# haiciyang/LaDiffCodec

Hardware: AMD Instinct MI355X
Metric: audio-sec decoded / wall-sec, 16kHz 3kbps 50-step DDPM (higher is better)
Workload: dtype bf16; 1 GPU; LaDiffCodec 3 kbps, diff_dims=256, enc_ratios 8 4, 50-step DDPM, batch=32x2.4 s utterances per GPU; global_batch=32, latent_len=1200, denoise_steps=50, rccl_ranks=1, batches_in_flight=1, parallelism=dp1 (utterance-sharded, no data-path collective)

## Files before the change

ladiffcodec_amd/csrc/conv_lean.inc:

```

struct LeanTile { int m0, n0, sk_k, sk_tile, R_lo, nrows, u_begin, u_end; };
struct LeanGeom {
  const LeanTile* tiles;
  unsigned long long* stamps;
  int debug;
  int ln_off;
  int grid;
};

enum { LEAN_K3 = 0, LEAN_K1 = 1, LEAN_K1_LN = 2, LEAN_K4S2 = 3, LEAN_K7 = 4 };
enum { LEAN_EPI_PLAIN = 0, LEAN_EPI_RES = 1, LEAN_EPI_GN = 2, LEAN_EPI_GN_RES = 3, LEAN_EPI_QKV = 4 };

template <int TM, int KIND, bool RF>
struct LeanShape {
  static constexpr bool K3 = KIND == LEAN_K3, K4 = KIND == LEAN_K4S2, K7 = KIND == LEAN_K7;
  static constexpr bool TAPS = K3 || K4 || K7;
  static constexpr int TG = K3 ? 3 : (TAPS ? 4 : 1), KC = TAPS ? 1 : 2, NS = TG * KC, NSB = NS + (RF ? 1 : 0);
  static constexpr int NTAP = K7 ? 8 : TG;
  static constexpr int BM = TM * 64, BN = 64;
  static constexpr int PLANE_ROWS = K4 ? (TM == 2 ? 272 : 144) : (TAPS ? (TM == 2 ? 144 : 80) : BM);
  static constexpr int NAW = (PLANE_ROWS / 16 + 3) / 4;
  static constexpr int NAW0 = NAW > 3 ? 3 : NAW, NAW1 = NAW - NAW0;
  static constexpr int PLANE_BYTES = PLANE_ROWS * kRowBytes + kRowBytes;
  static constexpr int ZERO_OFF = PLANE_ROWS * kRowBytes;
  static constexpr int B_OFF = KC * PLANE_BYTES;
  static constexpr int STAGE_BYTES = B_OFF + NSB * BN * kRowBytes;
  static_assert(NAW >= 1 && NAW <= 5 && NAW1 <= 2 && NSB >= 2 && NSB <= 4, "runs of at most four copies per M0 write (13-bit immediate)");
};

template <int N>
__device__ __forceinline__ void lean_dma_run(const char* base, unsigned m0v, unsigned cnt, unsigned v0, unsigned v1, unsigned v2) {
  if constexpr (N == 1) {
    if (cnt != 0u) asm volatile("s_mov_b32 m0, %2\n\ts_nop 0\n\tglobal_load_lds_dwordx4 %0, %1" ::"v"(v0), "s"(base), "s"(m0v) : "memory");
  } else if constexpr (N == 2) {
    asm volatile("s_mov_b32 m0, %3\n\ts_cmp_lt_u32 %4, 1\n\ts_cbranch_scc1 .Lq%=\n\tglobal_load_lds_dwordx4 %0, %2\n\t"
                 "s_cmp_lt_u32 %4, 2\n\ts_cbranch_scc1 .Lq%=\n\tglobal_load_lds_dwordx4 %1, %2 offset:1024\n.Lq%=:"
                 ::"v"(v0), "v"(v1), "s"(base), "s"(m0v), "s"(cnt) : "memory", "scc");
  } else {
    asm volatile("s_mov_b32 m0, %4\n\ts_cmp_lt_u32 %5, 1\n\ts_cbranch_scc1 .Lq%=\n\tglobal_load_lds_dwordx4 %0, %3\n\t"
                 "s_cmp_lt_u32 %5, 2\n\ts_cbranch_scc1 .Lq%=\n\tglobal_load_lds_dwordx4 %1, %3 offset:1024\n\t"
                 "s_cmp_lt_u32 %5, 3\n\ts_cbranch_scc1 .Lq%=\n\tglobal_load_lds_dwordx4 %2, %3 offset:2048\n.Lq%=:"
                 ::"v"(v0), "v"(v1), "v"(v2), "s"(base), "s"(m0v), "s"(cnt) : "memory", "scc");
  }
}
template <int N>
__device__ __forceinline__ void lean_dma_all(const char* base, unsigned m0v, unsigned v0, unsigned v1, unsigned v2, unsigned v3) {
  if constexpr (N == 2) {
    asm volatile("s_mov_b32 m0, %3\n\ts_nop 0\n\tglobal_load_lds_dwordx4 %0, %2\n\tglobal_load_lds_dwordx4 %1, %2 offset:1024"
                 ::"v"(v0), "v"(v1), "s"(base), "s"(m0v) : "memory");
  } else if constexpr (N == 3) {
    asm volatile("s_mov_b32 m0, %4\n\ts_nop 0\n\tglobal_load_lds_dwordx4 %0, %3\n\tglobal_load_lds_dwordx4 %1, %3 offset:1024\n\t"
                 "global_load_lds_dwordx4 %2, %3 offset:2048"
                 ::"v"(v0), "v"(v1), "v"(v2), "s"(base), "s"(m0v) : "memory");
  } else {
    asm volatile("s_mov_b32 m0, %5\n\ts_nop 0\n\tglobal_load_lds_dwordx4 %0, %4\n\tglobal_load_lds_dwordx4 %1, %4 offset:1024\n\t"
                 "global_load_lds_dwordx4 %2, %4 offset:2048\n\tglobal_load_lds_dwordx4 %3, %4 offset:3072"
                 ::"v"(v0), "v"(v1), "v"(v2), "v"(v3), "s"(base), "s"(m0v) : "memory");
  }
}


__device__ __forceinline__ float lean_wave_sum(float v) {
  auto dpp = [](float x, auto ctrl) { return __int_as_float(__builtin_amdgcn_update_dpp(0, __float_as_int(x), decltype(ctrl)::value, 0xf, 0xf, true)); };
  v += dpp(v, std::integral_constant<int, 0xB1>());
  v += dpp(v, std::integral_constant<int, 0x4E>());
  v += dpp(v, std::integral_constant<int, 0x141>());
  v += dpp(v, std::integral_constant<int, 0x140>());
  const int iv = __float_as_int(v);
  return (__int_as_float(__builtin_amdgcn_readlane(iv, 0)) + __int_as_float(__builtin_amdgcn_readlane(iv, 16))) +
         (__int_as_float(__builtin_amdgcn_readlane(iv, 32)) + __int_as_float(__builtin_amdgcn_readlane(iv, 48)));
}

template <int G>
__device__ __forceinline__ float lean_group_sum(float v) {
  static_assert(G == 4 || G == 8, "quad or half row");
  auto dpp = [](float x, auto ctrl) { return __int_as_float(__builtin_amdgcn_update_dpp(0, __float_as_int(x), decltype(ctrl)::value, 0xf, 0xf, true)); };
  v += dpp(v, std::integral_constant<int, 0xB1>());
  v += dpp(v, std::integral_constant<int, 0x4E>());
  if constexpr (G == 8) v += dpp(v, std::integral_constant<int, 0x141>());
// ... 327 lines not shown
  const int b_first = (int)fdiv((unsigned)m0, a.lrows_div);
  const int b_last = (int)fdiv((unsigned)(min(m0 + BM, M) - 1), a.lrows_div);
  for (int bb = b_first; bb <= b_last; ++bb) {
    const int lo = bb * a.L_rows, hi = min(lo + a.L_rows, M);
    float ps = 0.f;
#pragma unroll
    for (int i = 0; i < TM; ++i)
#pragma unroll
      for (int r = 0; r < 16; ++r) {
        const int rl = (wm * TM + i) * 32 + (r & 3) + 8 * (r >> 2) + 4 * g;
        const int m = m0 + rl;
        const bool in = m >= lo && m < hi;
        if (wn == 0) {
          const unsigned short pb = in ? hw_bf16(__expf(fminf(acc[i][0][r], kLinattnKClamp))) : (unsigned short)0;
          ps += __uint_as_float((unsigned)pb << 16);
          spT[i32 * P + rl] = pb;
        } else {
          svT[i32 * P + rl] = in ? hw_bf16(acc[i][0][r]) : (unsigned short)0;
        }
      }
    float* wsb = a.qkv_ctx_ws + (size_t)bb * a.qkv_ctx_stride;
    if (wn == 0) {
      ps += __shfl_xor(ps, 32);
      if (lane < 32) atomicAdd(&wsb[HD + head * D + i32], ps);
    }
    __syncthreads();
    if (wave == 0) {
      f32x16 c;
#pragma unroll
      for (int r = 0; r < 16; ++r) c[r] = 0.f;
#pragma unroll
      for (int sx = 0; sx < BM / 16; ++sx) {
        const uint4 pa = *reinterpret_cast<const uint4*>(&spT[i32 * P + 16 * sx + 8 * g]);
        const uint4 vb = *reinterpret_cast<const uint4*>(&svT[i32 * P + 16 * sx + 8 * g]);
        mfma_step<__bf16>(c, pa, vb);
      }
      float* ctx = wsb + 2 * HD + (size_t)head * D * D;
#pragma unroll
      for (int r = 0; r < 16; ++r) {
        const int d = (r & 3) + 8 * (r >> 2) + 4 * g;
        atomicAdd(&ctx[d * D + i32], c[r]);
      }
    }
    __syncthreads();
  }
}

typedef const __attribute__((address_space(3))) u32x4_t* lds_u4_cptr;
__device__ __forceinline__ uint4 lean_lds16(unsigned addr) {
  const u32x4_t v = *reinterpret_cast<lds_u4_cptr>(addr);
  return make_uint4(v[0], v[1], v[2], v[3]);
}

template <typename T, int TM, int KIND, bool RF, int EPI, bool SK, int S = 2>
__global__ __launch_bounds__(256, S == 3 ? 2 : 3) void conv_lean_kernel(const ConvKArgs a, const LeanGeom g) {
  using SH = LeanShape<TM, KIND, RF>;
  static_assert(S == 2 || (S == 3 && !SH::K4 && !SH::K7 && SH::NAW1 == 0), "three stages: the k = 3 and 1x1 kinds (one window run per plane)");
  constexpr int TN = 1, WM = 2, WN = 2, NW = 4, TG = SH::TG, KC = SH::KC, NS = SH::NS, NSB = SH::NSB, NAW = SH::NAW;
  constexpr int BM = SH::BM, BN = SH::BN, STAGE = SH::STAGE_BYTES, PLANE = SH::PLANE_BYTES;
  constexpr int BKE = kRowBytes / (int)sizeof(T);
  constexpr bool LN = KIND == LEAN_K1_LN;
  constexpr unsigned kBias = 3072u;
  static_assert(!RF || SH::K3, "the folded 1x1 conv rides on a k = 3 unit");
  static_assert((!SH::K4 && !SH::K7) || (EPI <= LEAN_EPI_RES && (!SK || SH::K4)), "k = 4 / 7: plain and residual epilogues; k = 7 is never split");
  extern __shared__ __attribute__((aligned(16))) char smem[];
  typedef __attribute__((address_space(3))) void* lptr_t;
  const unsigned lds_base = (unsigned)(size_t)(lptr_t)smem;

  const int tid = (int)threadIdx.x, lane = tid & 63;
  const int wave = __builtin_amdgcn_readfirstlane(tid >> 6);
  const int wm = wave >> 1, wn = wave & 1;
  const unsigned bid = blockIdx.x;
  unsigned long long t_start = 0, t_pro = 0, t_loop = 0, t_tab = 0, t_dma = 0;
  GnStamp gst = {0ull, 0ull, 0ull, 0u};
  if (g.stamps) t_start = __builtin_amdgcn_s_memtime();
  unsigned long long* kst_slot = nullptr;
  if (a.kst) {
    kst_slot = a.kst + (size_t)(a.kst_step[1] & 2047) * a.kst_stride;
    if (tid == 0 && bid == 0) kst_slot[0] = (unsigned long long)wall_clock64();
  }
  if (g.debug & 8) return;
  typedef const __attribute__((address_space(4))) LeanTile* tile_cptr;
  const tile_cptr tp = (tile_cptr)(unsigned long long)g.tiles + bid;
  LeanTile tl;
  tl.m0 = tp->m0; tl.n0 = tp->n0; tl.sk_k = tp->sk_k; tl.sk_tile = tp->sk_tile; tl.R_lo = tp->R_lo; tl.nrows = tp->nrows; tl.u_begin = tp->u_begin; tl.u_end = tp->u_end;
  const int M = a.B * a.L_rows;
  const int m0 = tl.m0, n0 = tl.n0, R_lo = tl.R_lo, nrows = tl.nrows;

  const int r16 = lane >> 2;
  const unsigned gslot = (unsigned)(((lane & 3) ^ ((r16 >> 2) & 3)) << 4);
  const unsigned ldb1 = (unsigned)a.C1 * (unsigned)sizeof(T), ldb2 = (unsigned)a.C2 * (unsigned)sizeof(T);
  unsigned vw[NAW];
  auto window_offsets = [&](const unsigned ldb) {
#pragma unroll
    for (int i = 0; i < NAW; ++i) {
      int r = (wave * NAW + i) * 16 + r16;
      if (r >= nrows) r = 0;
      vw[i] = (unsigned)(R_lo + r) * ldb + gslot + kBias - (unsigned)(i < SH::NAW0 ? i : i - SH::NAW0) * 1024u;
    }
  };
  const unsigned wcnt = (unsigned)__builtin_amdgcn_readfirstlane(max(0, min(NAW, (nrows - wave * NAW * 16 + 15) >> 4)));
  const unsigned slab_bytes = (unsigned)a.n_pad * kRowBytes;
  unsigned vb[4] = {0u, 0u, 0u, 0u};
#pragma unroll
  for (int q = 0; q < NSB; ++q) {
    const unsigned slab = SH::TAPS ? (unsigned)q * slab_bytes : (unsigned)q * (unsigned)a.wtaps * slab_bytes;
    vb[q] = slab + (unsigned)(n0 + wave * 16 + r16) * kRowBytes + gslot + kBias - (unsigned)q * 1024u;
  }
  const int csw = a.C1 / BKE;
  const int pc0 = SH::K7 ? tl.u_begin >> 1 : tl.u_begin * KC;
  int pc = pc0;
  const char* xb;
  if (pc0 >= csw && a.C2 > 0) {
    xb = a.x2 + (size_t)(pc0 - csw) * kRowBytes - kBias;
    window_offsets(ldb2);
  } else {
    xb = a.x1 + (size_t)pc0 * kRowBytes - kBias;
    window_offsets(ldb1);
  }
  const unsigned chunk_w = (unsigned)a.wtaps * slab_bytes;
  const char* wb = a.w + (size_t)pc0 * chunk_w - kBias;
  const unsigned m0_win = lds_base + (unsigned)(wave * NAW * 1024);
  const unsigned m0_b = lds_base + (unsigned)(SH::B_OFF + wave * NSB * 1024);
  if (g.stamps) t_tab = __builtin_amdgcn_s_memtime();

  const unsigned wcnt0 = SH::NAW1 ? min(wcnt, (unsigned)SH::NAW0) : wcnt, wcnt1 = wcnt - wcnt0;
  auto issue = [&](const int st) {
#pragma unroll
    for (int kc = 0; kc < KC; ++kc) {
      lean_dma_run<SH::NAW0>(xb + kc * kRowBytes, m0_win + (unsigned)(st * STAGE + kc * PLANE), wcnt0, vw[0], vw[NAW > 1 ? 1 : 0], vw[NAW > 2 ? 2 : 0]);
      if constexpr (SH::NAW1 > 0)
        lean_dma_run<SH::NAW1>(xb + kc * kRowBytes, m0_win + (unsigned)(st * STAGE + kc * PLANE + SH::NAW0 * 1024), wcnt1, vw[NAW > 3 ? 3 : 0], vw[NAW > 4 ? 4 : 0], 0u);
    }
    if constexpr (SH::K7) {
      if (st == 0) {
        lean_dma_all<4>(wb, m0_b + (unsigned)(st * STAGE), vb[0], vb[1], vb[2], vb[3]);
        wb += (size_t)4 * slab_bytes;
        return;
      }
      lean_dma_all<4>(wb, m0_b + (unsigned)(st * STAGE), vb[0], vb[1], vb[2], vb[3] - 3u * slab_bytes);
    } else {
      lean_dma_all<NSB>(wb, m0_b + (unsigned)(st * STAGE), vb[0], vb[1], vb[2], vb[3]);
    }
    pc += KC;
    xb += KC * kRowBytes;
    wb += SH::K7 ? (size_t)3 * slab_bytes : (size_t)KC * chunk_w;
    if (pc == csw) {
      xb = a.x2 - kBias;
      window_offsets(ldb2);
    }
  };
  issue(0);
  if constexpr (S == 3) {
    if (tl.u_begin + 1 < tl.u_end && !(g.debug & 16)) issue(1);
  }
  if (g.stamps) t_dma = __builtin_amdgcn_s_memtime();
  LeanCols cl = {0.f, 0.f, 0.f, 1.f, 0.f};
  auto fetch_cols = [&]() {
    const int ecol = n0 + wn * 32 + (lane & 31);
    const bool ok = ecol < a.n;
    const int cc = ok ? ecol : 0;
    if (a.bias && ok) cl.bias = a.bias[ecol];
    if constexpr (EPI == LEAN_EPI_GN || EPI == LEAN_EPI_GN_RES) {
      cl.gam = a.gn_gamma[cc]; cl.bet = a.gn_beta[cc];
      if (a.gn_ss) { cl.sc = a.gn_ss[cc] + 1.0f; cl.sh = a.gn_ss[a.n + cc]; }
    }
  };
  if constexpr (!RF) fetch_cols();

  if constexpr (LN) {
    constexpr int TPR = NW * 64 / BM;
    constexpr int EPV = 16 / (int)sizeof(T);
    const int row = tid / TPR, part = tid - row * TPR;
    const int C = a.C1, nvec = C / EPV;
    const char* src = a.x1 + (size_t)min(m0 + row, M - 1) * C * sizeof(T);
    float sm = 0.f, sq = 0.f;
    const float2* rs = a.ln_rowstat ? reinterpret_cast<const float2*>(a.ln_rowstat) + (size_t)min(m0 + row, M - 1) * (C >> 5) : nullptr;
    auto reduce_tpr = [&](float v) {
#pragma unroll
      for (int o = 1; o < TPR; o <<= 1) v += __shfl_xor(v, o);
      return v;
    };
    if (rs) {
      const int nblk = C >> 5;
      for (int k0 = part; k0 < nblk; k0 += TPR * 4) {
        float2 pr[4];
#pragma unroll
        for (int u = 0; u < 4; ++u) pr[u] = rs[min(k0 + u * TPR, nblk - 1)];
#pragma unroll
        for (int u = 0; u < 4; ++u)
          if (k0 + u * TPR < nblk) sm += pr[u].x;
      }
      const float mean = reduce_tpr(sm) / (float)C;
      for (int k0 = part; k0 < nblk; k0 += TPR * 4) {
        float2 pr[4];
#pragma unroll
        for (int u = 0; u < 4; ++u) pr[u] = rs[min(k0 + u * TPR, nblk - 1)];
#pragma unroll
        for (int u = 0; u < 4; ++u)
          if (k0 + u * TPR < nblk) {
            const float d = pr[u].x * (1.0f / 32.0f) - mean;
            sq += fmaf(32.0f * d, d, pr[u].y);
          }
      }
      sm = mean;
    } else {
      float mean = 0.f;
#pragma unroll 1
      for (int pass = 0; pass < 2; ++pass) {
        for (int v0 = part; v0 < nvec; v0 += TPR * 8) {
          uint4 q[8];
#pragma unroll
          for (int u = 0; u < 8; ++u) {
            const int v = v0 + u * TPR;
            q[u] = *reinterpret_cast<const uint4*>(src + (size_t)min(v, nvec - 1) * 16);
          }
#pragma unroll
          for (int u = 0; u < 8; ++u) {
            if (v0 + u * TPR >= nvec) continue;
            const unsigned w4[4] = {q[u].x, q[u].y, q[u].z, q[u].w};
#pragma unroll
            for (int e = 0; e < 4; ++e) {
              if (sizeof(T) == 4) {
                const float f = __uint_as_float(w4[e]);
                if (pass == 0) sm += f;
                else sq = fmaf(f - mean, f - mean, sq);
              } else {
                const float f0 = __uint_as_float(w4[e] << 16), f1 = __uint_as_float(w4[e] & 0xffff0000u);
                if (pass == 0) sm += f0 + f1;
                else sq = fmaf(f0 - mean, f0 - mean, fmaf(f1 - mean, f1 - mean, sq));
              }
            }
          }
        }
        if (pass == 0) mean = reduce_tpr(sm) / (float)C;
      }
      sm = mean;
    }
    sq = reduce_tpr(sq);
    if (part == 0) {
      float* st = reinterpret_cast<float*>(smem + g.ln_off);
      st[2 * row] = sm;
      st[2 * row + 1] = rsqrtf(sq / (float)C + 1e-5f);
    }
  }

  if (tid < S * KC * 16) {
    const int st = tid / (KC * 16), rem = tid - st * (KC * 16);
    reinterpret_cast<unsigned*>(smem + st * STAGE + (rem >> 4) * PLANE + SH::ZERO_OFF)[rem & 15] = 0u;
  }
  const int kh = lane >> 5;
  const int leff = a.L_in << a.ups;
  unsigned a_ad[TM][SH::NTAP][2];
#pragma unroll
  for (int i = 0; i < TM; ++i) {
    const int m = m0 + (wm * TM + i) * 32 + (lane & 31);
    int rb = -1, rl = 0;
    if (m < M) {
      rb = (int)fdiv((unsigned)m, a.lrows_div);
      rl = m - rb * a.L_rows;
    }
    const int u0 = rl * a.stride - a.pad_left;
    const int rowb = rb * a.L_in - R_lo;
#pragma unroll
    for (int t = 0; t < SH::NTAP; ++t) {
      const int u = u0 + t * a.dil;
      const bool ok = rb >= 0 && (unsigned)u < (unsigned)leff && (!SH::K7 || t < 7);
      const int row = rowb + (u >> a.ups);
      const int sw = (row >> 2) & 3;
      a_ad[i][t][0] = lds_base + (unsigned)(ok ? row * kRowBytes + ((kh ^ sw) << 4) : SH::ZERO_OFF);
      a_ad[i][t][1] = lds_base + (unsigned)(ok ? row * kRowBytes + (((2 + kh) ^ sw) << 4) : SH::ZERO_OFF);
    }
  }
  unsigned b_ad[2];
  {
    const int nl = wn * 32 + (lane & 31);
    const int rowb = ((nl >> 4) * NSB) * 16 + (nl & 15);
    const int sw = ((nl & 15) >> 2) & 3;
    b_ad[0] = lds_base + (unsigned)(SH::B_OFF + rowb * kRowBytes + ((kh ^ sw) << 4));
    b_ad[1] = lds_base + (unsigned)(SH::B_OFF + rowb * kRowBytes + (((2 + kh) ^ sw) << 4));
  }

  f32x16 acc[TM][TN];
#pragma unroll
  for (int i = 0; i < TM; ++i)
#pragma unroll
    for (int r = 0; r < 16; ++r) acc[i][0][r] = 0.0f;
  f32x16 acc2[RF ? TM : 1][1];
  if constexpr (RF) {
#pragma unroll
    for (int i = 0; i < TM; ++i)
#pragma unroll
      for (int r = 0; r < 16; ++r) acc2[i][0][r] = 0.0f;
  }

  auto compute = [&](const int st) {
#pragma unroll
    for (int q = 0; q < NS; ++q) {
      const int kc = q / TG, t = SH::K7 ? st * TG + q : q % TG;
#pragma unroll
// ... 58 lines not shown
#pragma unroll
        for (int ks = 0; ks < 2; ++ks)
#pragma unroll
          for (int i = 0; i < TM; ++i) {
            if constexpr (RF) {
              if (q == NS) { mfma_step<T>(acc2[i][0], af[q & 1][ks][i], bf[q & 1][ks]); continue; }
            }
            mfma_step<T>(acc[i][0], af[q & 1][ks][i], bf[q & 1][ks]);
          }
        if (pf) {
          __builtin_amdgcn_sched_barrier(0);
#pragma unroll
          for (int p = 0; p < NP; ++p)
            if (p == q || (q == NG - 1 && p > q)) piece(sti, p);
          __builtin_amdgcn_sched_barrier(0);
        }
      }
    };
    auto wait_keep_one = [&]() {
      if (NAW >= 3 && wcnt == 3u) asm volatile("s_waitcnt vmcnt(%0)" ::"n"(3 * KC + NSB) : "memory");
      else if (NAW >= 2 && wcnt == 2u) asm volatile("s_waitcnt vmcnt(%0)" ::"n"(2 * KC + NSB) : "memory");
      else if (wcnt == 1u) asm volatile("s_waitcnt vmcnt(%0)" ::"n"(KC + NSB) : "memory");
      else asm volatile("s_waitcnt vmcnt(%0)" ::"n"(NSB) : "memory");
    };
    auto handover = [&]() {
      asm volatile("s_waitcnt lgkmcnt(0)" ::: "memory");
      __builtin_amdgcn_s_barrier();
      asm volatile("" ::: "memory");
    };
    while (u + 3 < u_end) {
      wait_keep_one(); handover();
      step(0, 2, copies);
      wait_keep_one(); handover();
      step(1, 0, copies);
      wait_keep_one(); handover();
      step(2, 1, copies && u + 4 < u_end);
      u += 3;
    }
    const int left = u_end - u;
    if (left >= 1) {
      if (left >= 2) wait_keep_one(); else asm volatile("s_waitcnt vmcnt(0)" ::: "memory");
      handover();
      step(0, 2, copies && left >= 3);
    }
    if (left >= 2) {
      if (left >= 3) wait_keep_one(); else asm volatile("s_waitcnt vmcnt(0)" ::: "memory");
      handover();
      step(1, 0, false);
    }
    if (left >= 3) {
      asm volatile("s_waitcnt vmcnt(0)" ::: "memory");
      handover();
      step(2, 1, false);
    }
    u = u_end;
  }
  while (u + 1 < u_end) {
    asm volatile("s_waitcnt vmcnt(0)" ::: "memory");
    __syncthreads();
    if (copies) issue(1);
    compute(0);
    asm volatile("s_waitcnt vmcnt(0)" ::: "memory");
    __syncthreads();
    if (u + 2 < u_end && copies) issue(0);
    compute(1);
    u += 2;
  }
  if (u < u_end) {
    asm volatile("s_waitcnt vmcnt(0)" ::: "memory");
    __syncthreads();
    compute(0);
  }
  if (g.stamps) t_loop = __builtin_amdgcn_s_memtime();
  __syncthreads();

  if constexpr (SK) {
    int* s_last_p = reinterpret_cast<int*>(smem);
    constexpr int TILE = BM * BN;
    const int sk_tile = tl.sk_tile, sk_k = tl.sk_k;
    float* mine = a.sk_part + ((size_t)sk_tile * a.ksplit + sk_k) * TILE;
#pragma unroll
    for (int i = 0; i < TM; ++i)
#pragma unroll
      for (int r = 0; r < 16; ++r)
        __hip_atomic_store(&mine[((wave * TM + i) * 16 + r) * 64 + lane], acc[i][0][r], __ATOMIC_RELAXED, __HIP_MEMORY_SCOPE_AGENT);
    asm volatile("s_waitcnt vmcnt(0)" ::: "memory");
    __syncthreads();
    if (tid == 0) {
      const unsigned old = atomicAdd(a.sk_count + sk_tile, 1u);
      const int last = old == (unsigned)(a.ksplit - 1);
      *s_last_p = last;
      if (last) a.sk_count[sk_tile] = 0u;
    }
    __syncthreads();
    const int is_last = *s_last_p;
    __syncthreads();
    if (!is_last) return;
#pragma unroll
    for (int i = 0; i < TM; ++i)
#pragma unroll
      for (int r = 0; r < 16; ++r) acc[i][0][r] = 0.0f;
    for (int o = 0; o < a.ksplit; ++o) {
      const float* other = a.sk_part + ((size_t)sk_tile * a.ksplit + o) * TILE;
#pragma unroll
      for (int i = 0; i < TM; ++i)
#pragma unroll
// ... 194 lines not shown
      lean_tile_of(b, a, gm, BM, BN, t.m0, t.n0, t.sk_k, t.sk_tile);
    }
    int lo = 0, hi = 0;
    lean_tile_window(a, t.m0, BM, M, lo, hi);
    t.R_lo = lo;
    t.nrows = hi - lo + 1;
    mx = std::max(mx, t.nrows);
    t.u_begin = a.ksplit > 1 ? (int)(((long long)nunits_all * t.sk_k) / a.ksplit) : 0;
    t.u_end = a.ksplit > 1 ? (int)(((long long)nunits_all * (t.sk_k + 1)) / a.ksplit) : nunits_all;
  }
  return mx;
}

static const LeanTile* lean_tile_table(const ConvKArgs& a, const FastGeom& gm, int BM, int BN, int KC, int M, int bke, int* max_rows, int upc = 1) {
  struct Entry { LeanTile* dev; int max_rows; };
  static std::map<LeanKey, Entry> cache;
  static std::mutex mu;
  LeanKey k;
  memset(&k, 0, sizeof(k));
  const int vals[24] = {gm.grid, gm.ntiles, gm.ntn, gm.ntm, a.ksplit, gm.sk_xcd, gm.item_major, gm.m_fastest, BM, BN, KC, M, a.B, a.L_rows, a.L_in,
                        a.stride, a.taps, a.dil, a.pad_left, a.ups, a.reflect_back, a.reflect_fwd, a.C1 + a.C2, bke};
  memcpy(k.v, vals, sizeof(vals));
  int dev_id = 0;
  (void)hipGetDevice(&dev_id);
  k.v[23] = bke | (dev_id << 8);
  k.v[24] = a.wtaps * 65536 + a.n_pad;
  k.v[25] = a.tune ? a.tune->xcd_order : 0;
  k.v[26] = upc;
  std::lock_guard<std::mutex> lock(mu);
  auto it = cache.find(k);
  if (it != cache.end()) { *max_rows = it->second.max_rows; return it->second.dev; }
  std::vector<LeanTile> h;
  const int mx = lean_build_tiles(a, gm, BM, BN, KC, M, bke, upc, h);
  void* d = nullptr;
  if (hipMalloc(&d, h.size() * sizeof(LeanTile)) != hipSuccess) return nullptr;
  if (hipMemcpy(d, h.data(), h.size() * sizeof(LeanTile), hipMemcpyHostToDevice) != hipSuccess) { (void)hipFree(d); return nullptr; }
  cache[k] = Entry{(LeanTile*)d, mx};
  *max_rows = mx;
  return (LeanTile*)d;
}

template <typename T, int TM, int KIND, bool RF, int EPI, bool SK, int S = 2>
static hipError_t launch_lean_kernel(const ConvKArgs& a, const LeanGeom& g, size_t lds, hipStream_t s) {
  auto kern = conv_lean_kernel<T, TM, KIND, RF, EPI, SK, S>;
  static bool lds_opt_in = false;
  if (!lds_opt_in) {
    hipError_t e = hipFuncSetAttribute(reinterpret_cast<const void*>(kern), hipFuncAttributeMaxDynamicSharedMemorySize, 160 * 1024);
    if (e != hipSuccess) return e;
    lds_opt_in = true;
  }
  hipLaunchKernelGGL(kern, dim3(g.grid), dim3(256), lds, s, a, g);
  __atomic_fetch_add(&g_lean_launches[KIND], 1ll, __ATOMIC_RELAXED);
  if (S == 3) __atomic_fetch_add(&g_lean_launches[5], 1ll, __ATOMIC_RELAXED);
  return hipGetLastError();
}

template <typename T, int TM, bool RF>
static int lean_ring3_wgs_per_cu() {
  static int cached = -1;
  static std::mutex mu;
  std::lock_guard<std::mutex> lock(mu);
  if (cached >= 0) return cached;
  using SH = LeanShape<TM, LEAN_K3, RF>;
  int worst = 1 << 30;
  auto ask = [&](const void* fn, bool res32) {
    const size_t lds = std::max((size_t)3 * SH::STAGE_BYTES, (size_t)4 * TM * 32 * (32 * (res32 ? 4 : sizeof(T)) + 16));
    int n = 0;
    if (hipFuncSetAttribute(fn, hipFuncAttributeMaxDynamicSharedMemorySize, 160 * 1024) != hipSuccess ||
        hipOccupancyMaxActiveBlocksPerMultiprocessor(&n, fn, 256, lds) != hipSuccess) {
      (void)hipGetLastError();
      n = 0;
    }
    worst = std::min(worst, n);
  };
  ask(reinterpret_cast<const void*>(conv_lean_kernel<T, TM, LEAN_K3, RF, LEAN_EPI_GN, false, 3>), false);
  if constexpr (!RF) {
    ask(reinterpret_cast<const void*>(conv_lean_kernel<T, TM, LEAN_K3, false, LEAN_EPI_GN, true, 3>), false);
    ask(reinterpret_cast<const void*>(conv_lean_kernel<T, TM, LEAN_K3, false, LEAN_EPI_GN_RES, false, 3>), true);
    ask(reinterpret_cast<const void*>(conv_lean_kernel<T, TM, LEAN_K3, false, LEAN_EPI_GN_RES, true, 3>), true);
  }
  cached = worst;
  return cached;
}

template <typename T, int TM, int TG, int KC, bool RF>
static hipError_t launch_lean(const ConvKArgs& a, const FastGeom& gm, int M, hipStream_t s, bool* launched) {
  *launched = false;
  if constexpr (kW8 || kFp8 || !((TG == 3 && KC == 1) || (TG == 1 && KC == 2) || (TG == 4 && KC == 1 && sizeof(T) == 2)) || (RF && TG != 3)) {
    return hipSuccess;
  } else if constexpr (TG == 4) {
    const ConvTune* tn = a.tune;
    if (tn && (!tn->lean || !tn->lean_all)) return hipSuccess;
    const bool k4 = a.taps == 4 && a.stride == 2 && gm.ngroups == 1, k7 = a.taps == 7 && a.stride == 1 && gm.ngroups == 2;
    if (!(k4 || k7) || a.dil != 1 || a.ups || a.wtaps != a.taps) return hipSuccess;
    if (a.pad_mode != PAD_ZERO || a.post_act != ACT_NONE || a.gn_sum || a.gn_part || a.colmax || a.wscale || a.ln_s || a.qkv_ctx_ws || a.y2) return hipSuccess;
    constexpr int bke = kRowBytes / (int)sizeof(T);
    if ((a.C1 % bke) || (a.C2 % bke)) return hipSuccess;
    const bool sk = a.ksplit > 1, res = a.residual != nullptr;
    if (sk && (res || k7)) return hipSuccess;
    using SH4 = LeanShape<TM, LEAN_K4S2, false>;
    using SH7 = LeanShape<TM, LEAN_K7, false>;
    int max_rows = 0;
    const LeanTile* tiles = lean_tile_table(a, gm, SH4::BM, SH4::BN, 1, M, bke, &max_rows, k7 ? 2 : 1);
    if (!tiles) return hipErrorOutOfMemory;
    if (max_rows > (k4 ? SH4::PLANE_ROWS : SH7::PLANE_ROWS)) return hipSuccess;
    LeanGeom g;
    g.tiles = tiles; g.stamps = gm.stamps; g.debug = gm.debug; g.grid = gm.grid; g.ln_off = 0;
    const size_t epi_bytes = (size_t)4 * TM * 32 * (32 * (res ? 4 : sizeof(T)) + 16);
    const size_t lds = std::max((size_t)2 * (k4 ? SH4::STAGE_BYTES : SH7::STAGE_BYTES), epi_bytes);
    *launched = true;
    if (k4) {
      if (res) return launch_lean_kernel<T, TM, LEAN_K4S2, false, LEAN_EPI_RES, false>(a, g, lds, s);
      if (sk) return launch_lean_kernel<T, TM, LEAN_K4S2, false, LEAN_EPI_PLAIN, true>(a, g, lds, s);
      return launch_lean_kernel<T, TM, LEAN_K4S2, false, LEAN_EPI_PLAIN, false>(a, g, lds, s);
    }
    if (res) return launch_lean_kernel<T, TM, LEAN_K7, false, LEAN_EPI_RES, false>(a, g, lds, s);
    return launch_lean_kernel<T, TM, LEAN_K7, false, LEAN_EPI_PLAIN, false>(a, g, lds, s);
  } else {
    constexpr bool K3 = TG == 3;
    const ConvTune* tn = a.tune;
    if (tn && !tn->lean) return hipSuccess;
    if (gm.ngroups != 1 || a.pad_mode != PAD_ZERO || a.post_act != ACT_NONE || a.gn_sum || (K3 && a.colmax) || a.wscale) return hipSuccess;
    constexpr int bke = kRowBytes / (int)sizeof(T);
    if ((a.C1 % (bke * KC)) || (a.C2 % (bke * KC))) return hipSuccess;
    const bool gn = a.gn_part != nullptr;
    const bool res32 = a.residual != nullptr || (gn && (a.gn_out & 1));
    const int epi = gn ? (res32 ? LEAN_EPI_GN_RES : LEAN_EPI_GN) : (a.residual ? LEAN_EPI_RES : LEAN_EPI_PLAIN);
    const bool sk = a.ksplit > 1;
    const bool ln = a.ln_s != nullptr;
    if (ln && (K3 || sk || epi != LEAN_EPI_PLAIN)) return hipSuccess;
    const bool qctx = a.qkv_ctx_ws != nullptr;
    if (qctx && (!ln || sizeof(T) != 2 || a.n != 384 || a.colmax)) return hipErrorInvalidValue;
    if (RF && (epi != LEAN_EPI_GN || sk)) return hipSuccess;
    if (gn && ((a.L_rows + (TM * 64) - 1) / (TM * 64) + 1) * 2 * (a.gn_cpg >> 5) > 128) return hipSuccess;
    if (sk && epi == LEAN_EPI_RES) return hipSuccess;
    if (!K3 && (epi == LEAN_EPI_GN || epi == LEAN_EPI_GN_RES)) return hipSuccess;
    using SH0 = LeanShape<TM, K3 ? LEAN_K3 : LEAN_K1, RF>;
    int max_rows = 0;
    const LeanTile* tiles = lean_tile_table(a, gm, SH0::BM, SH0::BN, KC, M, bke, &max_rows);
    if (!tiles) return hipErrorOutOfMemory;
    if (max_rows > SH0::PLANE_ROWS) return hipSuccess;
    LeanGeom g;
    g.tiles = tiles; g.stamps = gm.stamps; g.debug = gm.debug; g.grid = gm.grid; g.ln_off = 0;
    const size_t epi_bytes = (size_t)4 * TM * 32 * (32 * ((epi == LEAN_EPI_RES || epi == LEAN_EPI_GN_RES) ? 4 : sizeof(T)) + 16);
    const size_t lds3 = std::max((size_t)3 * SH0::STAGE_BYTES, epi_bytes) + (ln ? (size_t)SH0::BM * 8 + 16 : 0);
    bool ring3 = tn && tn->ring3_tiles > 0 && gm.grid <= tn->ring3_tiles && (size_t)std::max(1, tn->ring3_wgs) * lds3 <= (size_t)160 * 1024 && !(gm.debug & 1);
    if (ring3 && gn) {
      const long slots = (long)lean_ring3_wgs_per_cu<T, TM, RF>() * tn->ring3_cu_share;
      const long item_tiles = (long)((a.L_rows + SH0::BM - 1) / SH0::BM + 1) * gm.ntn;
      ring3 = gm.grid <= slots || item_tiles + 16 * gm.ntn <= slots;
    }
    size_t lds = std::max((size_t)(ring3 ? 3 : 2) * SH0::STAGE_BYTES, epi_bytes);
    if (ln) {
      g.ln_off = (int)((lds + 15) / 16 * 16);
      lds = (size_t)g.ln_off + (size_t)SH0::BM * 8;
    }
    *launched = true;
#define LDC_LEAN_GO(KIND_, EPI_, SK_)                                                         \
  do {                                                                                        \
    if (ring3) return launch_lean_kernel<T, TM, KIND_, RF, EPI_, SK_, 3>(a, g, lds, s);       \
    return launch_lean_kernel<T, TM, KIND_, RF, EPI_, SK_, 2>(a, g, lds, s);                  \
  } while (0)
    if constexpr (K3) {
      if constexpr (RF) {
        LDC_LEAN_GO(LEAN_K3, LEAN_EPI_GN, false);
      } else {
        if (epi == LEAN_EPI_PLAIN) { if (sk) LDC_LEAN_GO(LEAN_K3, LEAN_EPI_PLAIN, true); LDC_LEAN_GO(LEAN_K3, LEAN_EPI_PLAIN, false); }
        if (epi == LEAN_EPI_RES) LDC_LEAN_GO(LEAN_K3, LEAN_EPI_RES, false);
        if (epi == LEAN_EPI_GN) { if (sk) LDC_LEAN_GO(LEAN_K3, LEAN_EPI_GN, true); LDC_LEAN_GO(LEAN_K3, LEAN_EPI_GN, false); }
        if (sk) LDC_LEAN_GO(LEAN_K3, LEAN_EPI_GN_RES, true);
        LDC_LEAN_GO(LEAN_K3, LEAN_EPI_GN_RES, false);
      }
    } else {
      if constexpr (sizeof(T) == 2) {
        if (qctx) LDC_LEAN_GO(LEAN_K1_LN, LEAN_EPI_QKV, false);
      }
      if (ln) LDC_LEAN_GO(LEAN_K1_LN, LEAN_EPI_PLAIN, false);
      if (epi == LEAN_EPI_RES) LDC_LEAN_GO(LEAN_K1, LEAN_EPI_RES, false);
      if (sk) LDC_LEAN_GO(LEAN_K1, LEAN_EPI_PLAIN, true);
      LDC_LEAN_GO(LEAN_K1, LEAN_EPI_PLAIN, false);
    }
#undef LDC_LEAN_GO
  }
}
```

ladiffcodec_amd/csrc/ldc_api.cpp:

```cpp
#include "ldc_internal.h"

long long g_device_syncs = 0;

static thread_local char g_err[1024] = "";
int fail(int code, const char* fmt, ...) {
  va_list ap;
  va_start(ap, fmt);
  vsnprintf(g_err, sizeof(g_err), fmt, ap);
  va_end(ap);
  return code;
}

extern "C" const char* ldc_last_error(void) { return g_err; }
extern "C" const char* ldc_version(void) { return "ladiffcodec-amd 0.1 (gfx950)"; }



static std::vector<float> fold_weight_norm(const HostTensor& g, const HostTensor& v) {
  const size_t n0 = (size_t)v.shape[0], inner = v.numel() / n0;
  std::vector<float> w(v.numel());
  for (size_t i = 0; i < n0; ++i) {
    double s = 0;
    for (size_t j = 0; j < inner; ++j) s += (double)v.data[i * inner + j] * v.data[i * inner + j];
    const float nrm = (float)sqrt(s);
// ... 747 lines not shown
      if (c->lstm_ev[k][e]) (void)hipEventDestroy(c->lstm_ev[k][e]);
  }
  for (auto& e : c->flow_ev) if (e) (void)hipEventDestroy(e);
  for (int k = 1; k < kMaxParts; ++k) {
    if (c->ev_join[k]) (void)hipEventDestroy(c->ev_join[k]);
    if (c->aux_stream[k]) (void)hipStreamDestroy(c->aux_stream[k]);
  }
  for (int k = 0; k < kMaxParts; ++k) {
    if (c->ev_side_fork[k]) (void)hipEventDestroy(c->ev_side_fork[k]);
    if (c->ev_side_join[k]) (void)hipEventDestroy(c->ev_side_join[k]);
    if (c->side_stream[k]) (void)hipStreamDestroy(c->side_stream[k]);
  }
  if (c->own_stream) (void)hipStreamDestroy(c->own_stream);
  delete c;
  return LDC_OK;
}

extern "C" void ldc_quantize_e4m3(const float* in, int64_t n, uint8_t* out_codes, float* out_values) {
  for (int64_t i = 0; i < n; ++i) {
    const uint8_t q = host_f32_to_e4m3(in[i]);
    if (out_codes) out_codes[i] = q;
    if (out_values) out_values[i] = host_e4m3_to_f32(q);
  }
}

struct OptRef { int* p; bool replan; int lo, hi; };
static bool find_option(ldc_ctx* c, const std::string& n, OptRef* r) {
#define LDC_OPT(NAME, FIELD, REPLAN, LO, HI) if (n == NAME) { r->p = &(FIELD); r->replan = REPLAN; r->lo = LO; r->hi = HI; return true; }
  LDC_OPT("split", c->split_batch, true, 1, kMaxParts)
  LDC_OPT("part_graphs", c->part_graphs, false, 0, 2)
  LDC_OPT("graph_steps", c->graph_steps, false, 0, 1000)
  LDC_OPT("flow_depth", c->flow_depth, false, 0, (int)ldc_ctx::kFlowRing - 1)
  LDC_OPT("split_ends", c->split_ends, false, 0, 1)
  LDC_OPT("ends_join", c->ends_join, false, 0, 1)
  LDC_OPT("split_init", c->split_init, true, 0, 1)
  LDC_OPT("side_streams", c->side_streams, true, 0, 1)
  LDC_OPT("serial_parts", c->serial_parts, false, 0, 1)
  LDC_OPT("stream_calib", c->calib, false, 0, 1)
  LDC_OPT("merge_advance", c->merge_advance, true, 0, 1)
  LDC_OPT("fuse_gn_stats", c->fuse_gn_stats, true, 0, 1)
  LDC_OPT("fuse_gn_epi", c->fuse_gn_epi, true, 0, 1)
  LDC_OPT("gn_epi_min_l", c->gn_epi_min_l, true, 0, 1 << 30)
  LDC_OPT("gn_epi_max_tiles", c->gn_epi_max_tiles, true, 0, 1 << 30)
  LDC_OPT("fold_res", c->fold_res, true, 0, 1)
  LDC_OPT("fold_ln", c->fold_ln, true, 0, 1)
  LDC_OPT("fuse_kmax", c->fuse_kmax, true, 0, 1)
  LDC_OPT("fuse_ln", c->fuse_ln, true, 0, 1)
  LDC_OPT("fuse_attn_tail", c->fuse_attn_tail, true, 0, 1)
  LDC_OPT("fold_ctx", c->fold_ctx, true, 0, 1)
  LDC_OPT("conv_lean", c->tune.lean, true, 0, 1)
  LDC_OPT("lean_all", c->tune.lean_all, true, 0, 1)
  LDC_OPT("ring3_tiles", c->tune.ring3_tiles, true, 0, 1 << 30)
  LDC_OPT("ring3_wgs", c->tune.ring3_wgs, true, 1, 3)
  LDC_OPT("conv_generic", c->tune.force_generic, true, 0, 1)
  LDC_OPT("conv_small_tiles", c->tune.small_max, true, 0, 1 << 30)
  LDC_OPT("conv_splitk", c->tune.splitk, true, 0, 4)
  LDC_OPT("sk_tiles", c->tune.sk_tiles, true, 0, 1 << 30)
  LDC_OPT("sk_u2", c->tune.sk_u2, true, 0, 1 << 30)
  LDC_OPT("sk_u3", c->tune.sk_u3, true, 0, 1 << 30)
  LDC_OPT("conv_mfast", c->tune.m_fastest, true, 0, 2)
  LDC_OPT("conv_debug", c->tune.debug, true, 0, 255)
  LDC_OPT("conv_tile", c->tune.force_tile, true, -1, 1)
  LDC_OPT("conv_xcd_order", c->tune.xcd_order, true, 0, 8)
  LDC_OPT("gn_nap", c->tune.gn_nap, true, 0, 4096)
  LDC_OPT("gn_nap0", c->tune.gn_nap0, true, 0, 4096)
  LDC_OPT("lstm_stream", c->lstm_stream_only, false, 0, 1)
  LDC_OPT("lstm_xcd", c->lstm_xcd, false, 0, 1)
  LDC_OPT("lstm_pipe", c->lstm_pipe, false, 0, 1)
  LDC_OPT("coop_launch", c->coop_launch, false, 0, 1)
  LDC_OPT("sea_splitk", c->sea_splitk, false, 0, 1)
  LDC_OPT("rvq_tiled", c->rvq_tiled, false, 0, 1)
  LDC_OPT("train_bf16", g_train_bf16, false, 0, 1)
  LDC_OPT("train_fp32_mfma", g_train_fp32_mfma, false, 0, 1)
  LDC_OPT("train_valu", g_train_valu, false, 0, 1)
  LDC_OPT("train_dw_side", g_train_dw_side, false, 0, 1)
#undef LDC_OPT
  return false;
}

extern "C" int ldc_set_option(ldc_ctx* c, const char* name, int value) {
  if (!c || !name) return fail(LDC_E_INVALID, "null context or option name");
  const std::string n(name);
  if (n == "fp8_act") {
    if (c->finalized) return fail(LDC_E_STATE, "fp8_act must be set before ldc_finalize_weights");
    c->fp8_act = value ? 1 : 0;
    return LDC_OK;
  }
  if (n == "plan_cache_gb") { c->plan_bytes_cap = (size_t)std::max(1, value) << 30; return LDC_OK; }
  if (n == "plan_cache_n") { c->plan_count_cap = std::max(2 * kMaxParts, value); return LDC_OK; }
  OptRef r;
  if (!find_option(c, n, &r)) return fail(LDC_E_INVALID, "unknown option '%s' (tools/README.md lists the options)", name);
  if (value < r.lo || value > r.hi) return fail(LDC_E_INVALID, "option %s must be in %d..%d", name, r.lo, r.hi);
  if (n == "side_streams" && value && c->split_batch != 1) return fail(LDC_E_INVALID, "side streams need a single chain (split 1)");
  if (value == *r.p) return LDC_OK;
  if (r.replan && c->live_pools > 0)
    return fail(LDC_E_STATE, "option %s rebuilds every plan, and %d decode pool(s) keep their items' state in theirs: destroy the pools first", name, c->live_pools);
  if (r.replan && !c->plans.empty()) { HIPCHK(hipSetDevice(c->device)); drop_plans(c); }
  *r.p = value;
  if (n == "split" && value != 1) c->side_streams = 0;
  return LDC_OK;
}

extern "C" long long ldc_debug_sync_count(void) { return g_device_syncs; }

extern "C" int ldc_debug_raise_failure(ldc_ctx* c, int code) {
  if (!c || !c->dev_flag_host || (code != 1 && code != 2 && code != (int)kDevFailCtxRange)) return fail(LDC_E_INVALID, "bad arguments");
// ... 1498 lines not shown
```

ladiffcodec_amd/csrc/ldc_kernels.h:

```cpp
#pragma once
#include <hip/hip_runtime.h>
#include <stdint.h>

#include "ldc_windows.h"

namespace ldc {

enum { DT_F32 = 0, DT_BF16 = 1, DT_FP8 = 2 };
enum { ACT_NONE = 0, ACT_SILU = 1, ACT_ELU = 2, ACT_TANH = 3, ACT_GELU = 4, ACT_SIGMOID = 5, ACT_RELU = 6 };
enum { PAD_ZERO = 0, PAD_REFLECT = 1 };
static constexpr int kGnPad = 16;

inline size_t dt_size(int dt) { return dt == DT_F32 ? 4 : (dt == DT_FP8 ? 1 : 2); }

struct ConvLayer {
  int dt = DT_F32;
  int cin1 = 0, cin2 = 0;
  int n = 0;
  int n_pad = 0;
  int bn = 128;
  int taps = 1, stride = 1, dil = 1, pad_left = 0, ups = 0, pad_mode = PAD_ZERO;
  int pre_act = ACT_NONE, post_act = ACT_NONE;
  int tr_stride = 0, tr_cout = 0, tr_trim_left = 0;
  void* w = nullptr;
  float* bias = nullptr;
  int w8 = 0;
  float* wscale = nullptr;
  double flops_per_row = 0;
  float* ln_s = nullptr;
  int wtaps = 0;
  float* bias2 = nullptr;
};

struct ConvTune {
  int force_generic = 0;
  int small_max = 100;
  int splitk = 1;
  int sk_tiles = 200, sk_u2 = 24, sk_u3 = 60;
  int m_fastest = 1;
  int debug = 0;
  int gn_nap = 16, gn_nap0 = 0;
  int force_tile = -1;
  int xcd_order = 1;
  int lean = 1;
  int ring3_tiles = 304;
  int ring3_wgs = 3;
  int ring3_cu_share = 102;
  int lean_all = 1;
};

struct ConvCall {
  const void* x1 = nullptr;
  const void* x2 = nullptr;
  void* y = nullptr;
  void* y2 = nullptr;
  const void* residual = nullptr;
  int B = 0;
  int L_in = 0;
  int L_rows = 0;
  int L_final = 0;
  int y_ld = 0;
  float* gn_sum = nullptr;
  int gn_groups = 0;
  unsigned* colmax = nullptr;
  int colmax_lo = 0, colmax_hi = 0, colmax_stride = 0;
  float* qkv_ctx_ws = nullptr;
  int qkv_ctx_stride = 0;
  float* sk_part = nullptr;
  unsigned* sk_count = nullptr;
  long long sk_part_cap = 0;
  int sk_count_cap = 0;
  int generic_split = 0;
  void* gn_part = nullptr;
  int gn_mslots = 0;
  const float* gn_gamma = nullptr;
  const float* gn_beta = nullptr;
  const float* gn_ss = nullptr;
  int gn_out = 0;
  unsigned* fail_flag = nullptr;
  float* rowstat_out = nullptr;
  const float* ln_rowstat = nullptr;
  unsigned long long* kst = nullptr;
  const int* kst_step = nullptr;
  int kst_stride = 0;
  const void* ctx = nullptr;
  const int* ctx_fresh = nullptr;
  int ctx_rows = 0, ctx_zero = 0;
  int check_only = 0;
  const ConvTune* tune = nullptr;
  long long* sk_need = nullptr;
  int* route_out = nullptr;
  int* bm_out = nullptr;
};

enum { CONV_ROUTE_NONE = 0, CONV_ROUTE_CIN1_ROWS = 1, CONV_ROUTE_CIN1_GENERIC = 2, CONV_ROUTE_PIPELINED = 3, CONV_ROUTE_GENERIC = 4 };
hipError_t launch_conv(const ConvLayer& ly, const ConvCall& c, hipStream_t s);
long long conv_generic_splitk_floats(const ConvLayer& ly, const ConvCall& c);
size_t conv_packed_weight_bytes(const ConvLayer& ly);
void pack_conv_weights(const ConvLayer& ly, const float* w_oik, void* dst_host);
// ... 234 lines not shown
```

Before: 633.8 audio-s/wall-s.

## Add three-slot window ring with double-buffered weight slabs for k=3 lean convs

Adds a new pipeline variant for the k = 3 lean conv kernel. Input windows rotate through three LDS slots while the weight slabs use only two buffers, so the per-workgroup LDS footprint shrinks enough for three workgroups per CU where the full three-stage ring did not fit. Window and slab DMA issues are interleaved inside the MFMA loop. The host selects the variant when ring3 is rejected for LDS size and the grid is within a tile threshold, with an occupancy query for GN epilogues. This adds deeper prefetch at higher occupancy, at the cost of more complex waitcnt and barrier handling and extra template instantiations.

```diff
diff --git a/ladiffcodec_amd/csrc/conv_lean.inc b/ladiffcodec_amd/csrc/conv_lean.inc
--- a/ladiffcodec_amd/csrc/conv_lean.inc
+++ b/ladiffcodec_amd/csrc/conv_lean.inc
@@ -24,7 +24,9 @@
   static constexpr int PLANE_BYTES = PLANE_ROWS * kRowBytes + kRowBytes;
   static constexpr int ZERO_OFF = PLANE_ROWS * kRowBytes;
   static constexpr int B_OFF = KC * PLANE_BYTES;
-  static constexpr int STAGE_BYTES = B_OFF + NSB * BN * kRowBytes;
+  static constexpr int SLAB_BYTES = NSB * BN * kRowBytes;
+  static constexpr int STAGE_BYTES = B_OFF + SLAB_BYTES;
+  static constexpr int RINGW_BYTES = 3 * KC * PLANE_BYTES + 2 * SLAB_BYTES;
   static_assert(NAW >= 1 && NAW <= 5 && NAW1 <= 2 && NSB >= 2 && NSB <= 4, "runs of at most four copies per M0 write (13-bit immediate)");
 };
 
@@ -458,10 +460,15 @@
   return make_uint4(v[0], v[1], v[2], v[3]);
 }
 
+enum { LEAN_RING_W = 5 };
 template <typename T, int TM, int KIND, bool RF, int EPI, bool SK, int S = 2>
 __global__ __launch_bounds__(256, S == 3 ? 2 : 3) void conv_lean_kernel(const ConvKArgs a, const LeanGeom g) {
   using SH = LeanShape<TM, KIND, RF>;
-  static_assert(S == 2 || (S == 3 && !SH::K4 && !SH::K7 && SH::NAW1 == 0), "three stages: the k = 3 and 1x1 kinds (one window run per plane)");
+  constexpr bool RW = S == LEAN_RING_W;
+  static_assert(S == 2 || RW || (S == 3 && !SH::K4 && !SH::K7 && SH::NAW1 == 0), "three stages: the k = 3 and 1x1 kinds (one window run per plane)");
+  static_assert(!RW || (SH::K3 && SH::NAW1 == 0 && !RF), "window ring: k = 3 units (one plane, one window run), no folded second conv");
+  static_assert(!RW || 3 * std::max(SH::RINGW_BYTES, 4 * TM * 32 * (32 * ((EPI == LEAN_EPI_RES || EPI == LEAN_EPI_GN_RES) ? 4 : (int)sizeof(T)) + 16)) <= 160 * 1024,
+                "window ring: three workgroups of it (ring or epilogue staging, whichever is larger) fit a CU's 160 KB of LDS");
   constexpr int TN = 1, WM = 2, WN = 2, NW = 4, TG = SH::TG, KC = SH::KC, NS = SH::NS, NSB = SH::NSB, NAW = SH::NAW;
   constexpr int BM = SH::BM, BN = SH::BN, STAGE = SH::STAGE_BYTES, PLANE = SH::PLANE_BYTES;
   constexpr int BKE = kRowBytes / (int)sizeof(T);
@@ -556,9 +563,29 @@
       window_offsets(ldb2);
     }
   };
-  issue(0);
-  if constexpr (S == 3) {
-    if (tl.u_begin + 1 < tl.u_end && !(g.debug & 16)) issue(1);
+  constexpr unsigned kSlabs0 = (unsigned)(3 * PLANE - SH::B_OFF);
+  auto issue_window = [&](const int slot) {
+    lean_dma_run<SH::NAW0>(xb, m0_win + (unsigned)(slot * PLANE), wcnt, vw[0], vw[NAW > 1 ? 1 : 0], vw[NAW > 2 ? 2 : 0]);
+    pc += 1;
+    xb += kRowBytes;
+    if (pc == csw) {
+      xb = a.x2 - kBias;
+      window_offsets(ldb2);
+    }
+  };
+  auto issue_slabs = [&](const unsigned m0v) {
+    lean_dma_all<NSB>(wb, m0v, vb[0], vb[1], vb[2], vb[3]);
+    wb += (size_t)chunk_w;
+  };
+  if constexpr (RW) {
+    issue_window(0);
+    issue_slabs(m0_b + kSlabs0);
+    if (tl.u_begin + 1 < tl.u_end && !(g.debug & 16)) issue_window(1);
+  } else {
+    issue(0);
+    if constexpr (S == 3) {
+      if (tl.u_begin + 1 < tl.u_end && !(g.debug & 16)) issue(1);
+    }
   }
   if (g.stamps) t_dma = __builtin_amdgcn_s_memtime();
   LeanCols cl = {0.f, 0.f, 0.f, 1.f, 0.f};
@@ -651,7 +678,9 @@
     }
   }
 
-  if (tid < S * KC * 16) {
+  if constexpr (RW) {
+    if (tid < 3 * 16) reinterpret_cast<unsigned*>(smem + (tid >> 4) * PLANE + SH::ZERO_OFF)[tid & 15] = 0u;
+  } else if (tid < S * KC * 16) {
     const int st = tid / (KC * 16), rem = tid - st * (KC * 16);
     reinterpret_cast<unsigned*>(smem + st * STAGE + (rem >> 4) * PLANE + SH::ZERO_OFF)[rem & 15] = 0u;
   }
@@ -816,6 +845,75 @@
       asm volatile("s_waitcnt vmcnt(0)" ::: "memory");
       handover();
       step(2, 1, false);
+    }
+    u = u_end;
+  }
+  if constexpr (RW) {
+    constexpr int NG = NS;
+    unsigned bA[2] = {b_ad[0] + kSlabs0, b_ad[1] + kSlabs0}, bB[2] = {bA[0] + (unsigned)SH::SLAB_BYTES, bA[1] + (unsigned)SH::SLAB_BYTES};
+    unsigned mA = m0_b + kSlabs0, mB = mA + (unsigned)SH::SLAB_BYTES;
+    auto frag = [&](const int ws, const unsigned (&bx)[2], const int q, uint4 (&af)[2][TM], uint4 (&bf)[2]) {
+#pragma unroll
+      for (int ks = 0; ks < 2; ++ks) {
+#pragma unroll
+        for (int i = 0; i < TM; ++i) af[ks][i] = lean_lds16(a_ad[i][q][ks] + (unsigned)(ws * PLANE));
+        bf[ks] = lean_lds16(bx[ks] + (unsigned)(q * 1024));
+      }
+    };
+    auto step = [&](const int ws, const unsigned (&bx)[2], const unsigned m0n, const bool slabs, const bool window) {
+      uint4 af[2][2][TM], bf[2][2];
+      frag(ws, bx, 0, af[0], bf[0]);
+#pragma unroll
+      for (int q = 0; q < NG; ++q) {
+        if (q + 1 < NG) frag(ws, bx, q + 1, af[(q + 1) & 1], bf[(q + 1) & 1]);
+#pragma unroll
+        for (int ks = 0; ks < 2; ++ks)
+#pragma unroll
+          for (int i = 0; i < TM; ++i) mfma_step<T>(acc[i][0], af[q & 1][ks][i], bf[q & 1][ks]);
+        if ((q == 0 && slabs) || (q == 1 && window)) {
+          __builtin_amdgcn_sched_barrier(0);
+          if (q == 0) issue_slabs(m0n);
+          else issue_window((ws + 2) % 3);
+          __builtin_amdgcn_sched_barrier(0);
+        }
+      }
+    };
+    auto wait_keep_window = [&]() {
+      if (NAW >= 3 && wcnt == 3u) asm volatile("s_waitcnt vmcnt(3)" ::: "memory");
+      else if (NAW >= 2 && wcnt == 2u) asm volatile("s_waitcnt vmcnt(2)" ::: "memory");
+      else if (wcnt == 1u) asm volatile("s_waitcnt vmcnt(1)" ::: "memory");
+      else asm volatile("s_waitcnt vmcnt(0)" ::: "memory");
+    };
+    auto handover = [&]() {
+      asm volatile("s_waitcnt lgkmcnt(0)" ::: "memory");
+      __builtin_amdgcn_s_barrier();
+      asm volatile("" ::: "memory");
+    };
+    while (u + 3 < u_end) {
+      wait_keep_window(); handover();
+      step(0, bA, mB, copies, copies);
+      wait_keep_window(); handover();
+      step(1, bB, mA, copies, copies);
+      wait_keep_window(); handover();
+      step(2, bA, mB, copies, copies && u + 4 < u_end);
+      u += 3;
+      { const unsigned t0 = bA[0], t1 = bA[1], tm = mA; bA[0] = bB[0]; bA[1] = bB[1]; mA = mB; bB[0] = t0; bB[1] = t1; mB = tm; }
+    }
+    const int left = u_end - u;
+    if (left >= 1) {
+      if (left >= 2) wait_keep_window(); else asm volatile("s_waitcnt vmcnt(0)" ::: "memory");
+      handover();
+      step(0, bA, mB, copies && left >= 2, copies && left >= 3);
+    }
+    if (left >= 2) {
+      if (left >= 3) wait_keep_window(); else asm volatile("s_waitcnt vmcnt(0)" ::: "memory");
+      handover();
+      step(1, bB, mA, copies && left >= 3, false);
+    }
+    if (left >= 3) {
+      asm volatile("s_waitcnt vmcnt(0)" ::: "memory");
+      handover();
+      step(2, bA, mB, false, false);
     }
     u = u_end;
   }
@@ -1116,7 +1214,38 @@
   hipLaunchKernelGGL(kern, dim3(g.grid), dim3(256), lds, s, a, g);
   __atomic_fetch_add(&g_lean_launches[KIND], 1ll, __ATOMIC_RELAXED);
   if (S == 3) __atomic_fetch_add(&g_lean_launches[5], 1ll, __ATOMIC_RELAXED);
+  if (S == LEAN_RING_W) __atomic_fetch_add(&g_lean_launches[6], 1ll, __ATOMIC_RELAXED);
   return hipGetLastError();
+}
+
+template <int TM, int KIND, bool RF>
+struct LeanRingW { static constexpr bool ok = KIND == LEAN_K3 && TM == 2 && !RF; };
+
+template <typename T>
+static int lean_ringw_wgs_per_cu() {
+  constexpr int TM = 2;
+  static int cached = -1;
+  static std::mutex mu;
+  std::lock_guard<std::mutex> lock(mu);
+  if (cached >= 0) return cached;
+  using SH = LeanShape<TM, LEAN_K3, false>;
+  int worst = 1 << 30;
+  auto ask = [&](const void* fn, bool res32) {
+    const size_t lds = std::max((size_t)SH::RINGW_BYTES, (size_t)4 * TM * 32 * (32 * (res32 ? 4 : sizeof(T)) + 16));
+    int n = 0;
+    if (hipFuncSetAttribute(fn, hipFuncAttributeMaxDynamicSharedMemorySize, 160 * 1024) != hipSuccess ||
+        hipOccupancyMaxActiveBlocksPerMultiprocessor(&n, fn, 256, lds) != hipSuccess) {
+      (void)hipGetLastError();
+      n = 0;
+    }
+    worst = std::min(worst, n);
+  };
+  ask(reinterpret_cast<const void*>(conv_lean_kernel<T, TM, LEAN_K3, false, LEAN_EPI_GN, false, LEAN_RING_W>), false);
+  ask(reinterpret_cast<const void*>(conv_lean_kernel<T, TM, LEAN_K3, false, LEAN_EPI_GN, true, LEAN_RING_W>), false);
+  ask(reinterpret_cast<const void*>(conv_lean_kernel<T, TM, LEAN_K3, false, LEAN_EPI_GN_RES, false, LEAN_RING_W>), true);
+  ask(reinterpret_cast<const void*>(conv_lean_kernel<T, TM, LEAN_K3, false, LEAN_EPI_GN_RES, true, LEAN_RING_W>), true);
+  cached = worst;
+  return cached;
 }
 
 template <typename T, int TM, bool RF>
@@ -1214,7 +1343,18 @@
       const long item_tiles = (long)((a.L_rows + SH0::BM - 1) / SH0::BM + 1) * gm.ntn;
       ring3 = gm.grid <= slots || item_tiles + 16 * gm.ntn <= slots;
     }
-    size_t lds = std::max((size_t)(ring3 ? 3 : 2) * SH0::STAGE_BYTES, epi_bytes);
+    bool ringw = false;
+    if constexpr (LeanRingW<TM, K3 ? LEAN_K3 : LEAN_K1, RF>::ok) {
+      const size_t ldsw = std::max((size_t)SH0::RINGW_BYTES, epi_bytes);
+      ringw = !ring3 && tn && tn->ring3_window && gm.grid <= tn->ring3_window_tiles &&
+              (size_t)std::max(1, tn->ring3_wgs) * lds3 > (size_t)160 * 1024 && (size_t)std::max(1, tn->ring3_wgs) * ldsw <= (size_t)160 * 1024 && !(gm.debug & 1);
+      if (ringw && gn) {
+        const long slots = (long)lean_ringw_wgs_per_cu<T>() * tn->ring3_cu_share;
+        const long item_tiles = (long)((a.L_rows + SH0::BM - 1) / SH0::BM + 1) * gm.ntn;
+        ringw = gm.grid <= slots || item_tiles + 16 * gm.ntn <= slots;
+      }
+    }
+    size_t lds = std::max(ringw ? (size_t)SH0::RINGW_BYTES : (size_t)(ring3 ? 3 : 2) * SH0::STAGE_BYTES, epi_bytes);
     if (ln) {
       g.ln_off = (int)((lds + 15) / 16 * 16);
       lds = (size_t)g.ln_off + (size_t)SH0::BM * 8;
@@ -1222,6 +1362,9 @@
     *launched = true;
 #define LDC_LEAN_GO(KIND_, EPI_, SK_)                                                         \
   do {                                                                                        \
+    if constexpr (LeanRingW<TM, KIND_, RF>::ok) {                                             \
+      if (ringw) return launch_lean_kernel<T, TM, KIND_, RF, EPI_, SK_, LEAN_RING_W>(a, g, lds, s); \
+    }                                                                                         \
     if (ring3) return launch_lean_kernel<T, TM, KIND_, RF, EPI_, SK_, 3>(a, g, lds, s);       \
     return launch_lean_kernel<T, TM, KIND_, RF, EPI_, SK_, 2>(a, g, lds, s);                  \
   } while (0)
diff --git a/ladiffcodec_amd/csrc/ldc_api.cpp b/ladiffcodec_amd/csrc/ldc_api.cpp
--- a/ladiffcodec_amd/csrc/ldc_api.cpp
+++ b/ladiffcodec_amd/csrc/ldc_api.cpp
@@ -823,6 +823,8 @@
   LDC_OPT("lean_all", c->tune.lean_all, true, 0, 1)
   LDC_OPT("ring3_tiles", c->tune.ring3_tiles, true, 0, 1 << 30)
   LDC_OPT("ring3_wgs", c->tune.ring3_wgs, true, 1, 3)
+  LDC_OPT("ring3_window", c->tune.ring3_window, true, 0, 1)
+  LDC_OPT("ring3_window_tiles", c->tune.ring3_window_tiles, true, 0, 1 << 30)
   LDC_OPT("conv_generic", c->tune.force_generic, true, 0, 1)
   LDC_OPT("conv_small_tiles", c->tune.small_max, true, 0, 1 << 30)
   LDC_OPT("conv_splitk", c->tune.splitk, true, 0, 4)
diff --git a/ladiffcodec_amd/csrc/ldc_kernels.h b/ladiffcodec_amd/csrc/ldc_kernels.h
--- a/ladiffcodec_amd/csrc/ldc_kernels.h
+++ b/ladiffcodec_amd/csrc/ldc_kernels.h
@@ -45,6 +45,8 @@
   int lean = 1;
   int ring3_tiles = 304;
   int ring3_wgs = 3;
+  int ring3_window = 1;
+  int ring3_window_tiles = 608;
   int ring3_cu_share = 102;
   int lean_all = 1;
 };
```

Result: faster. 645.1 audio-s/wall-s (median of 6 runs) (+1.8%).
